# DefaultRui/VLN-VER

Measured on AMD Instinct MI355X. Metric: viewpoints/sec (multi-view->voxel fwd+bwd), vocc.py config, higher is better.
Workload: dtype bf16

## Files before the change

### vln-ver_amd/csrc/ver_wgrad.hip

```cpp
#include <cstdlib>
#include "ver_common.h"

namespace {
typedef __bf16 bf16x8 __attribute__((ext_vector_type(8)));
typedef float f32x16 __attribute__((ext_vector_type(16)));
typedef short s16x4 __attribute__((ext_vector_type(4)));
typedef short s16x8 __attribute__((ext_vector_type(8)));
typedef __attribute__((address_space(3))) s16x4 lds_s16x4;
typedef __attribute__((address_space(3))) void lds_void;

constexpr int kTile = 256;
constexpr int kSlabRows = 16;
constexpr int kSlabBytes = 2 * kSlabRows * kTile * 2;
constexpr int kRing = 8;
constexpr int kLdsBytes = kRing * kSlabBytes;

typedef int i32x2 __attribute__((ext_vector_type(2)));
typedef int i32x4 __attribute__((ext_vector_type(4)));

template <int OFF>
__device__ __forceinline__ i32x2 tr_read(int addr) {
    i32x2 v;
    asm volatile("ds_read_b64_tr_b16 %0, %1 offset:%2" : "=v"(v) : "v"(addr), "n"(OFF) : "memory");
    return v;
}
__device__ __forceinline__ bf16x8 frag(i32x2 lo, i32x2 hi) {
    return __builtin_bit_cast(bf16x8, (i32x4)__builtin_shufflevector(lo, hi, 0, 1, 2, 3));
}

struct WgradArgs {
    const __bf16* A;
    const __bf16* G;
    float* ws;
    long lda, ldg, M, Mc;
    int S, Ka, N, tiles_n, T;
    void* out;
    long ldo;
    int out_bf16;
    const __bf16* lattice;
    long lattice_bytes;
    const __bf16* cst;
    long cst_bytes;
    int B, H, W, C, P, CW, ncst, nseg;
    int seg_start[65];
    signed char kind[64], dz[64], dy[64], dx[64];
};

constexpr int kOutsideW = (int)0x80000000;
template <int L>
__device__ __forceinline__ int wcell_off(const WgradArgs& t, int b, int zl, int y, int x, int dz) {
    if ((unsigned)y >= (unsigned)t.H || (unsigned)x >= (unsigned)t.W) return kOutsideW;
    const int j = dz >> 1;
    int v;
    if (L == 0)
        v = ((b * 4 + zl + dz) * t.H + y) * t.W + x;
    else if (L == 2)
        v = ((((b * 2 + zl) * t.H + y) * t.W + x) << 1) + j;
    else
        v = (((((((y & 1) << 1 | (x & 1)) * t.B + b) * 2 + zl) * (t.H >> 1) + (y >> 1)) * (t.W >> 1) + (x >> 1)) << 1) + j;
    return v * t.C * 2;
}

struct WTapLane {
    int taddr;
    int boff;
    int bstep;
    int pend;
    int tend;
    int rows_left;
    int vo;
};

template <int L>
__device__ __forceinline__ int wtap_table_entry(const WgradArgs& t, int seg, int pos) {
    if (seg < 0) return kOutsideW;
    if (t.kind[seg]) return (pos * t.ncst + t.dz[seg]) * t.CW * 2;
    const int hw = t.H * t.W;
    const int zl = pos / hw, rem = pos - zl * hw;
    const int y = rem / t.W, x = rem - y * t.W;
    return wcell_off<L>(t, 0, zl, y + t.dy[seg], x + t.dx[seg], t.dz[seg]);
}

__device__ __forceinline__ int lds_read_b32(int addr) {
    int v;
    asm volatile("ds_read_b32 %0, %1" : "=v"(v) : "v"(addr) : "memory");
    return v;
}

__device__ __forceinline__ void wtap_step(const WgradArgs& t, WTapLane& tl, int tfetched) {
    tl.boff += tl.pend;
    tl.rows_left -= kSlabRows;
    tl.vo = tl.rows_left > 0 ? (int)((unsigned)tfetched + (unsigned)tl.boff) : kOutsideW;
    tl.taddr += 4 * kSlabRows;
    tl.pend = 0;
    if (tl.taddr >= tl.tend) tl.taddr -= 4 * t.P, tl.pend = tl.bstep;
}

struct WgradLane {
    int offA0, offA1, offB0, offB1;
    int voA, voG;
    int stepA, stepG;
    int dmaoff;
};

template <int SLOT>
__device__ __forceinline__ void read_slab(const WgradLane& c, i32x2 (&al)[4], i32x2 (&ah)[4], i32x2 (&bl)[2], i32x2 (&bh)[2]) {
    constexpr int SB = (SLOT & 3) * kSlabBytes;
    constexpr int UP = SLOT >= 4 ? 65536 : 0;
    const int a0 = c.offA0 + UP, a1 = c.offA1 + UP, b0 = c.offB0 + UP, b1 = c.offB1 + UP;
    al[0] = tr_read<SB>(a0);
    ah[0] = tr_read<SB + 512>(a0);
    bl[0] = tr_read<SB>(b0);
    bh[0] = tr_read<SB + 512>(b0);
    al[1] = tr_read<SB>(a1);
    ah[1] = tr_read<SB + 512>(a1);
    bl[1] = tr_read<SB>(b1);
    bh[1] = tr_read<SB + 512>(b1);
    al[2] = tr_read<SB + 1024>(a0);
    ah[2] = tr_read<SB + 1536>(a0);
    al[3] = tr_read<SB + 1024>(a1);
    ah[3] = tr_read<SB + 1536>(a1);
}

template <int PS, int KP, int PF, int IMPL>
__device__ __forceinline__ void phase(char* lds, f32x16 (&acc)[4][2], const WgradLane& c, __amdgpu_buffer_rsrc_t ra,
                                      __amdgpu_buffer_rsrc_t rg, unsigned& soA, unsigned& soG, const WgradArgs& t, WTapLane& tl) {
    i32x2 al[KP][4], ah[KP][4], bl[KP][2], bh[KP][2];
    int tnext = 0;
    read_slab<PS * KP>(c, al[0], ah[0], bl[0], bh[0]);
    if constexpr (KP == 2) read_slab<PS * KP + 1>(c, al[KP - 1], ah[KP - 1], bl[KP - 1], bh[KP - 1]);
#pragma unroll
    for (int u = 0; u < KP; ++u) {
        const int ds = (PS * KP + u + PF) % kRing;
        if constexpr (IMPL < 0) {
            __builtin_amdgcn_raw_ptr_buffer_load_lds(ra, (lds_void*)(lds + ds * kSlabBytes + c.dmaoff), 16, c.voA, (int)soA, 0, 0);
        } else {
            static_assert(IMPL < 0 || KP == 1, "implicit A: one slab per phase");
            __builtin_amdgcn_raw_ptr_buffer_load_lds(ra, (lds_void*)(lds + ds * kSlabBytes + c.dmaoff), 16, tl.vo, 0, 0, 0);
            tnext = lds_read_b32(tl.taddr);
        }
        __builtin_amdgcn_raw_ptr_buffer_load_lds(rg, (lds_void*)(lds + ds * kSlabBytes + kSlabBytes / 2 + c.dmaoff), 16, c.voG, (int)soG, 0, 0);
        soA += (unsigned)c.stepA;
        soG += (unsigned)c.stepG;
    }
    asm volatile("s_waitcnt vmcnt(%0)" ::"n"(2 * (PF - KP)) : "memory");
    __builtin_amdgcn_s_barrier();
    asm volatile("s_waitcnt lgkmcnt(0)"
                 : "+v"(al[0][0]), "+v"(ah[0][0]), "+v"(al[0][1]), "+v"(ah[0][1]), "+v"(al[0][2]), "+v"(ah[0][2]), "+v"(al[0][3]),
                   "+v"(ah[0][3]), "+v"(bl[0][0]), "+v"(bh[0][0]), "+v"(bl[0][1]), "+v"(bh[0][1]), "+v"(tnext)
                 :
                 : "memory");

    if constexpr (KP == 2)
        asm volatile(""
                     : "+v"(al[KP - 1][0]), "+v"(ah[KP - 1][0]), "+v"(al[KP - 1][1]), "+v"(ah[KP - 1][1]), "+v"(al[KP - 1][2]),
                       "+v"(ah[KP - 1][2]), "+v"(al[KP - 1][3]), "+v"(ah[KP - 1][3]), "+v"(bl[KP - 1][0]), "+v"(bh[KP - 1][0]),
                       "+v"(bl[KP - 1][1]), "+v"(bh[KP - 1][1])
                     :
                     : "memory");
    bf16x8 a[KP][4], b[KP][2];
#pragma unroll
    for (int u = 0; u < KP; ++u) {
#pragma unroll
        for (int i = 0; i < 4; ++i) a[u][i] = frag(al[u][i], ah[u][i]);
        b[u][0] = frag(bl[u][0], bh[u][0]);
        b[u][1] = frag(bl[u][1], bh[u][1]);
    }
    __builtin_amdgcn_sched_barrier(0);
    __builtin_amdgcn_s_setprio(1);
#pragma unroll
    for (int u = 0; u < KP; ++u)
#pragma unroll
        for (int it = 0; it < 4; ++it)
#pragma unroll
            for (int jt = 0; jt < 2; ++jt)
                acc[it][jt] = __builtin_amdgcn_mfma_f32_32x32x16_bf16(a[u][it], b[u][jt], acc[it][jt], 0, 0, 0);
    __builtin_amdgcn_s_setprio(0);
    __builtin_amdgcn_sched_barrier(0);
    if constexpr (IMPL >= 0) {
        wtap_step(t, tl, tnext);
        __builtin_amdgcn_sched_barrier(0);
    }
    __builtin_amdgcn_s_barrier();
}

template <int PS, int KP, int PF, int IMPL>
__device__ __forceinline__ void phases_from(int left, char* lds, f32x16 (&acc)[4][2], const WgradLane& c,
                                            __amdgpu_buffer_rsrc_t ra, __amdgpu_buffer_rsrc_t rg, unsigned& soA, unsigned& soG,
                                            const WgradArgs& t, WTapLane& tl) {
    if constexpr (PS < kRing / KP) {
        if (left > PS * KP) {
            phase<PS, KP, PF, IMPL>(lds, acc, c, ra, rg, soA, soG, t, tl);
            phases_from<PS + 1, KP, PF, IMPL>(left, lds, acc, c, ra, rg, soA, soG, t, tl);
        }
    }
}

template <int KP, int PF, int IMPL>
__device__ __forceinline__ void wgrad_body(const WgradArgs& p) {
    static_assert(PF >= KP && PF + (KP == 1 ? 2 : 4) <= kRing, "prefetch distance against the ring (WAR on the slot)");
    extern __shared__ __attribute__((aligned(1024))) char lds[];
    const int tid = threadIdx.x, lane = tid & 63;
    const int wave = __builtin_amdgcn_readfirstlane(tid >> 6);
    const int wr = wave >> 2, wc = wave & 3;
    int chunk, tile;
    {
        const int b = blockIdx.x;
        if ((p.S & 7) == 0) {
            const int xcd = b & 7, idx = b >> 3;
            chunk = xcd + 8 * (idx / p.T);
            tile = idx % p.T;
        } else {
            chunk = b / p.T;
            tile = b % p.T;
        }
    }
    const int mt = tile / p.tiles_n, nt = tile - mt * p.tiles_n;
    const long row0 = (long)chunk * p.Mc;
    const long rows = max(0L, min(p.Mc, p.M - row0));
    const int nslab = (int)((rows + kSlabRows * KP - 1) / (kSlabRows * KP)) * KP;

    const __bf16* ab = IMPL < 0 ? p.A + row0 * p.lda + (long)mt * kTile : nullptr;
    const __bf16* gb = p.G + row0 * p.ldg + (long)nt * kTile;
    const long abytes = ((p.M - row0 - 1) * p.lda + p.Ka - (long)mt * kTile) * 2;
    const long gbytes = ((p.M - row0 - 1) * p.ldg + p.N - (long)nt * kTile) * 2;
    const __amdgpu_buffer_rsrc_t rg = __builtin_amdgcn_make_buffer_rsrc((void*)gb, 0, (int)max(0L, min(gbytes, 0xFFFFFFFFL)), 0x00020000);
    WgradLane c;
    const int prow = lane >> 3, pch = (lane & 7) ^ (((prow >> 1) & 1) << 2);
    WTapLane tl = {};
    bool a_cst = false;
    if constexpr (IMPL >= 0) {
        int* tables = reinterpret_cast<int*>(lds + kLdsBytes);
        auto seg_of = [&](int col0) {
            int seg = -1;
            for (int i = 0; i < p.nseg; ++i)
                if (col0 >= p.seg_start[i] && col0 < p.seg_start[i + 1]) seg = i;
            return seg;
        };
        for (int q = 0; q < 4; ++q) {
            const int seg = seg_of(mt * kTile + 64 * q);
            for (int i = tid; i < p.P; i += 512) tables[q * p.P + i] = wtap_table_entry<IMPL>(p, seg, i);
        }
        __syncthreads();
        const int col0 = mt * kTile + 64 * (wave & 3);
        const int seg = seg_of(col0);
        a_cst = seg >= 0 && p.kind[seg];
        const long r = row0 + 8 * (wave >> 2) + prow;
        const int b0 = (int)(r / p.P), pos0 = (int)(r - (long)b0 * p.P);
        tl.bstep = a_cst ? 0 : (IMPL == 3 ? p.H * p.W : 4 * p.H * p.W) * p.C * 2;
        tl.boff = b0 * tl.bstep + (seg < 0 ? 0 : (col0 - p.seg_start[seg]) * 2) + pch * 16;
        const int lbase = (int)(uintptr_t)(__attribute__((address_space(3))) char*)(lds + kLdsBytes) + (wave & 3) * p.P * 4;
        tl.tend = lbase + 4 * p.P;
        tl.taddr = lbase + 4 * pos0;
        tl.pend = 0;
        tl.rows_left = (int)min(min(p.M, row0 + p.Mc) - r, 0x7FFFFFF0L) + kSlabRows;
        int t0 = lds_read_b32(tl.taddr);
        asm volatile("s_waitcnt lgkmcnt(0)" : "+v"(t0)::"memory");
        wtap_step(p, tl, t0);
    }
    const __amdgpu_buffer_rsrc_t ra =
        IMPL < 0 ? __builtin_amdgcn_make_buffer_rsrc((void*)ab, 0, (int)max(0L, min(abytes, 0xFFFFFFFFL)), 0x00020000)
                 : __builtin_amdgcn_make_buffer_rsrc((void*)(a_cst ? p.cst : p.lattice), 0,
                                                     (int)max(0L, min(a_cst ? p.cst_bytes : p.lattice_bytes, 0x7FFFFFFFL)), 0x00020000);
    c.voA = (int)(((8 * (wave >> 2) + prow) * p.lda + 64 * (wave & 3)) * 2) + pch * 16;
    c.voG = (int)(((8 * (wave >> 2) + prow) * p.ldg + 64 * (wave & 3)) * 2) + pch * 16;
    c.stepA = (int)(kSlabRows * p.lda * 2);
    c.stepG = (int)(kSlabRows * p.ldg * 2);
    c.dmaoff = wave * 1024;
    unsigned soA = 0, soG = 0;

    {
        const int q = lane >> 4, cl = lane & 15;
        const int lowch = (2 * (q & 1) + ((cl & 3) >> 1)) ^ (((cl >> 3) & 1) << 2);
        const int lbase = (int)(uintptr_t)(__attribute__((address_space(3))) char*)lds;
        const int rowoff = lbase + ((q >> 1) * 32 + (cl >> 2)) * 128 + lowch * 16 + (cl & 1) * 8;
        c.offA0 = rowoff + 2 * wr * 1024;
        c.offA1 = c.offA0 ^ 64;
        c.offB0 = rowoff + wc * 1024 + kSlabBytes / 2;
        c.offB1 = c.offB0 ^ 64;
    }

    f32x16 acc[4][2];
#pragma unroll
    for (int it = 0; it < 4; ++it)
#pragma unroll
        for (int jt = 0; jt < 2; ++jt)
#pragma unroll
            for (int r = 0; r < 16; ++r) acc[it][jt][r] = 0.0f;

#pragma unroll
    for (int s = 0; s < PF; ++s) {
        if constexpr (IMPL < 0) {
            __builtin_amdgcn_raw_ptr_buffer_load_lds(ra, (lds_void*)(lds + s * kSlabBytes + c.dmaoff), 16, c.voA, (int)soA, 0, 0);
        } else {
            __builtin_amdgcn_raw_ptr_buffer_load_lds(ra, (lds_void*)(lds + s * kSlabBytes + c.dmaoff), 16, tl.vo, 0, 0, 0);
            int tn = lds_read_b32(tl.taddr);
            asm volatile("s_waitcnt lgkmcnt(0)" : "+v"(tn)::"memory");
            wtap_step(p, tl, tn);
        }
        __builtin_amdgcn_raw_ptr_buffer_load_lds(rg, (lds_void*)(lds + s * kSlabBytes + kSlabBytes / 2 + c.dmaoff), 16, c.voG, (int)soG, 0, 0);
        soA += (unsigned)c.stepA;
        soG += (unsigned)c.stepG;
    }
    asm volatile("s_waitcnt vmcnt(%0)" ::"n"(2 * (PF - KP)) : "memory");
    __builtin_amdgcn_s_barrier();
    if (wr == 1) __builtin_amdgcn_s_barrier();

    int s = 0;
    for (; s + kRing <= nslab; s += kRing) phases_from<0, KP, PF, IMPL>(kRing, lds, acc, c, ra, rg, soA, soG, p, tl);
    phases_from<0, KP, PF, IMPL>(nslab - s, lds, acc, c, ra, rg, soA, soG, p, tl);
    if (wr == 0) __builtin_amdgcn_s_barrier();
    asm volatile("s_waitcnt vmcnt(0)" ::: "memory");

    const int i0 = mt * kTile + 128 * wr + 4 * (lane >> 5), j0 = nt * kTile + 64 * wc + (lane & 31);
    if (p.S == 1 && p.out) {
#pragma unroll
        for (int it = 0; it < 4; ++it)
#pragma unroll
            for (int jt = 0; jt < 2; ++jt) {
                const int j = j0 + 32 * jt;
#pragma unroll
                for (int r = 0; r < 16; ++r) {
                    const int i = i0 + 32 * it + (r & 3) + 8 * (r >> 2);
                    if (i < p.Ka && j < p.N) {
                        if (p.out_bf16)
                            reinterpret_cast<__bf16*>(p.out)[(long)i * p.ldo + j] = (__bf16)acc[it][jt][r];
                        else
                            reinterpret_cast<float*>(p.out)[(long)i * p.ldo + j] = acc[it][jt][r];
                    }
                }
            }
        return;
    }
    float* out = p.ws + (long)chunk * p.Ka * p.N;
#pragma unroll
    for (int it = 0; it < 4; ++it)
#pragma unroll
        for (int jt = 0; jt < 2; ++jt) {
            const int j = j0 + 32 * jt;
#pragma unroll
            for (int r = 0; r < 16; ++r) {
                const int i = i0 + 32 * it + (r & 3) + 8 * (r >> 2);
                if (i < p.Ka && j < p.N) out[(long)i * p.N + j] = acc[it][jt][r];
            }
        }
}

template <int KP, int PF>
__global__ __launch_bounds__(512) void k_wgrad_tn(WgradArgs p) {
    wgrad_body<KP, PF, -1>(p);
}

template <int L, int PF>
__global__ __launch_bounds__(512) void k_wgrad_tn_seg(WgradArgs p) {
    wgrad_body<1, PF, L>(p);
}

template <typename OT>
__global__ __launch_bounds__(256) void k_wgrad_reduce(const float* __restrict__ ws, OT* __restrict__ out, long ldo, int S,
                                                      int Ka, int N) {
    const long n4 = (long)Ka * N / 4;
    const long stride = (long)Ka * N;
    for (long e = blockIdx.x * 256L + threadIdx.x; e < n4; e += (long)gridDim.x * 256) {
        float4 acc = *reinterpret_cast<const float4*>(ws + 4 * e);
        for (int s = 1; s < S; ++s) {
            const float4 v = *reinterpret_cast<const float4*>(ws + s * stride + 4 * e);
            acc.x += v.x;
            acc.y += v.y;
            acc.z += v.z;
            acc.w += v.w;
        }
        const long i = (4 * e) / N, j = (4 * e) - i * N;
        OT* o = out + i * ldo + j;
        if constexpr (sizeof(OT) == 4) {
            *reinterpret_cast<float4*>(o) = acc;
        } else {
            typedef __bf16 bf16x4 __attribute__((ext_vector_type(4)));
            bf16x4 v;
            v.x = (__bf16)acc.x;
            v.y = (__bf16)acc.y;
            v.z = (__bf16)acc.z;
            v.w = (__bf16)acc.w;
            *reinterpret_cast<bf16x4*>(o) = v;
        }
    }
}

long max_chunk_rows(long ld) {
    if (ld <= 0) return 45000;
    const long rows = (0xFFFFFFFFL / (ld * 2)) - 16 * kRing - 2 * kSlabRows - 1;
    return rows < 45000 ? (rows > 2 * kSlabRows ? rows : 2 * kSlabRows) : 45000;
}

int pick_splits(long M, int Ka, int N, long ld = 0) {
    const long cap = max_chunk_rows(ld);
    const long tiles = (long)((Ka + kTile - 1) / kTile) * ((N + kTile - 1) / kTile);
    static const int cand[] = {1, 2, 3, 4, 6, 8, 12, 16, 24, 32, 48, 64};
    int best = 0;
    double best_us = 0.0;
    for (int s : cand) {
        if ((M + s - 1) / s > cap) continue;
        if (s > 1 && M / s < 256) break;
        if (M > 32768 && s % 8) continue;
        const long rounds = (tiles * s + 255) / 256;
        const double slabs = (double)((M + s - 1) / s + 15) / 16.0;
        double us = (double)rounds * (slabs * 0.37 + 8.0) + (s == 1 ? 0.25 : (double)s) * (double)Ka * (double)N * 8.0 / 3.0e6;
        if (s % 8 == 0) us *= 0.97;
        if (!best || us < best_us) {
            best = s;
            best_us = us;
        }
    }
    if (!best) {
        best = 64;
        while (best < 65536 && (M + best - 1) / best > cap) best *= 2;
    }
    return best;
}

template <int KP, int PF>
void launch_tn(const WgradArgs& p, int blocks, hipStream_t st, hipError_t& e) {
    auto kern = k_wgrad_tn<KP, PF>;
    e = hipFuncSetAttribute((const void*)kern, hipFuncAttributeMaxDynamicSharedMemorySize, kLdsBytes);
    if (e == hipSuccess) hipLaunchKernelGGL(kern, dim3((unsigned)blocks), dim3(512), kLdsBytes, st, p);
}
template <int L, int PF>
void launch_tn_segments_pf(const WgradArgs& p, int blocks, hipStream_t st, hipError_t& e) {
    const int ldsb = kLdsBytes + 4 * p.P * 4;
    e = hipFuncSetAttribute((const void*)k_wgrad_tn_seg<L, PF>, hipFuncAttributeMaxDynamicSharedMemorySize, ldsb);
    if (e == hipSuccess) hipLaunchKernelGGL((k_wgrad_tn_seg<L, PF>), dim3((unsigned)blocks), dim3(512), ldsb, st, p);
}

template <int L>
void launch_tn_segments(const WgradArgs& p, int blocks, hipStream_t st, hipError_t& e) {
    static const int pf = [] {
        const char* v = getenv("VER_WGRAD_SEG_PF");
        return v ? atoi(v) : 3;
    }();
    if (pf == 4) launch_tn_segments_pf<L, 4>(p, blocks, st, e);
    else if (pf == 5) launch_tn_segments_pf<L, 5>(p, blocks, st, e);
    else if (pf == 6) launch_tn_segments_pf<L, 6>(p, blocks, st, e);
    else launch_tn_segments_pf<L, 3>(p, blocks, st, e);
}
}

extern "C" int ver_wgrad_tn_splits(long M, int Ka, int N) {
    if (M <= 0 || Ka <= 0 || N <= 0) return 1;
    return pick_splits(M, Ka, N);
}

extern "C" int ver_wgrad_tn_splits_ld(long M, int Ka, int N, long ld) {
    if (M <= 0 || Ka <= 0 || N <= 0) return 1;
    return pick_splits(M, Ka, N, ld);
}

extern "C" long ver_wgrad_tn_workspace(long M, int Ka, int N, int splits) {
    if (Ka <= 0 || N <= 0) return 0;
    if (splits <= 0) splits = ver_wgrad_tn_splits(M, Ka, N);
    return (long)splits * Ka * N * (long)sizeof(float);
}

extern "C" int ver_wgrad_tn(const void* a, long lda, const void* g, long ldg, long M, int Ka, int N, void* out, long ldo,
                            int out_dtype, int splits, int flags, void* workspace, long workspace_bytes, void* stream) {
    hipStream_t st = (hipStream_t)stream;
    VER_REQUIRE(M >= 0 && Ka > 0 && N > 0, VER_EINVAL, "ver_wgrad_tn: bad sizes M=%ld Ka=%d N=%d", M, Ka, N);
    VER_REQUIRE(out && workspace && ((a && g) || M == 0), VER_EINVAL, "ver_wgrad_tn: null pointer argument");
    VER_REQUIRE(out_dtype == VER_F32 || out_dtype == VER_BF16, VER_EINVAL, "ver_wgrad_tn: out_dtype %d", out_dtype);
    VER_REQUIRE(lda >= Ka && ldg >= N && ldo >= N, VER_EINVAL, "ver_wgrad_tn: row pitch smaller than the row");
    VER_REQUIRE(lda % 8 == 0 && ldg % 8 == 0 && ((uintptr_t)a & 15) == 0 && ((uintptr_t)g & 15) == 0, VER_EUNSUPPORTED,
                "ver_wgrad_tn: operands must be 16-byte aligned with row pitches that are multiples of 8 elements");
    VER_REQUIRE(N % 4 == 0 && ldo % 4 == 0 && ((uintptr_t)out & 15) == 0, VER_EUNSUPPORTED,
                "ver_wgrad_tn: N and the output pitch must be multiples of 4");
    const int S = splits > 0 ? splits : pick_splits(M, Ka, N, lda > ldg ? lda : ldg);
    VER_REQUIRE(S <= 65536, VER_EINVAL, "ver_wgrad_tn: %d row chunks", S);
    const long Mc = ((M + S - 1) / S + 2 * kSlabRows - 1) / (2 * kSlabRows) * (2 * kSlabRows);
    VER_REQUIRE((Mc + 16 * kRing) * (lda > ldg ? lda : ldg) * 2 < 0xFFFFFFFFL, VER_EUNSUPPORTED,
                "ver_wgrad_tn: a row chunk exceeds the 4-GiB range of a buffer offset (more splits)");
    VER_REQUIRE(workspace_bytes >= (long)S * Ka * N * (long)sizeof(float), VER_EINVAL, "ver_wgrad_tn: workspace of %ld bytes, %ld needed",
                workspace_bytes, (long)S * Ka * N * (long)sizeof(float));
    WgradArgs p = {};
    p.A = (const __bf16*)a;
    p.G = (const __bf16*)g;
    p.ws = (float*)workspace;
    p.lda = lda;
    p.ldg = ldg;
    p.M = M;
    p.Mc = Mc;
    p.S = S;
    p.Ka = Ka;
    p.N = N;
    p.tiles_n = (N + kTile - 1) / kTile;
    p.T = ((Ka + kTile - 1) / kTile) * p.tiles_n;
    const bool direct = S == 1 && M > 0;
    p.out = direct ? out : nullptr;
    p.ldo = ldo;
    p.out_bf16 = out_dtype == VER_BF16;
    hipError_t e = hipSuccess;
    if (M > 0) {
        switch (flags & 15) {
            case 4: launch_tn<1, 4>(p, p.T * S, st, e); break;
            case 5: launch_tn<1, 5>(p, p.T * S, st, e); break;
            case 6: launch_tn<1, 6>(p, p.T * S, st, e); break;
            case 8 + 2: launch_tn<2, 2>(p, p.T * S, st, e); break;
            case 8 + 4: launch_tn<2, 4>(p, p.T * S, st, e); break;
            default: launch_tn<1, 3>(p, p.T * S, st, e); break;
        }
        if (e != hipSuccess) return ver_fail(VER_ELAUNCH, "ver_wgrad_tn: LDS attribute: %s", hipGetErrorString(e));
    } else if (int zrc = ver_zero_async(workspace, (size_t)S * Ka * N * sizeof(float), st)) {
        return zrc;
    }
    if (direct) return ver_check_launch("ver_wgrad_tn");
    const long n4 = (long)Ka * N / 4;
    long grid = (n4 + 255) / 256;
    if (grid > 8192) grid = 8192;
    if (out_dtype == VER_F32)
        hipLaunchKernelGGL(k_wgrad_reduce<float>, dim3((unsigned)grid), dim3(256), 0, st, (const float*)workspace, (float*)out, ldo, S, Ka, N);
    else
        hipLaunchKernelGGL(k_wgrad_reduce<__bf16>, dim3((unsigned)grid), dim3(256), 0, st, (const float*)workspace, (__bf16*)out, ldo, S, Ka, N);
    return ver_check_launch("ver_wgrad_tn");
}

extern "C" int ver_wgrad_tn_segments(const void* lattice, int layout, int B, int H, int W, int C, const int* taps, int nseg,
                                     const void* cst, int ncst, int cw, const void* g, long ldg, int N, void* out, long ldo,
                                     int out_dtype, int splits, void* workspace, long workspace_bytes, void* stream) {
    hipStream_t st = (hipStream_t)stream;
    VER_REQUIRE(B >= 0 && H > 0 && W > 0 && C > 0 && N > 0 && nseg > 0, VER_EINVAL, "ver_wgrad_tn_segments: bad sizes");
    VER_REQUIRE(layout == 0 || layout == 2 || layout == 3, VER_EINVAL, "ver_wgrad_tn_segments: layout %d (0 plain, 2 z-split, 3 planar z-split)", layout);
    VER_REQUIRE(layout != 3 || (H % 2 == 0 && W % 2 == 0), VER_EINVAL, "ver_wgrad_tn_segments: planar needs even H, W");
    VER_REQUIRE(out && workspace && ((lattice && g && taps) || B == 0), VER_EINVAL, "ver_wgrad_tn_segments: null pointer argument");
    VER_REQUIRE(out_dtype == VER_F32 || out_dtype == VER_BF16, VER_EINVAL, "ver_wgrad_tn_segments: out_dtype %d", out_dtype);
    VER_REQUIRE(nseg <= 64, VER_EUNSUPPORTED, "ver_wgrad_tn_segments: %d segments (at most 64)", nseg);
    VER_REQUIRE(C % 64 == 0 && (cst == nullptr || (ncst > 0 && ncst <= 64 && cw > 0 && cw % 64 == 0 && ((uintptr_t)cst & 15) == 0)),
                VER_EUNSUPPORTED, "ver_wgrad_tn_segments: segment widths (C = %d, pattern blocks of %d) must be multiples of 64", C, cw);
    const long M = (long)B * 2 * H * W, lbytes = (long)B * 4 * H * W * C * 2;
    const int P = 2 * H * W;
    VER_REQUIRE(P >= kSlabRows && P <= 2048 && lbytes < 0x7FFFFFFFL, VER_EUNSUPPORTED,
                "ver_wgrad_tn_segments: %d rows per viewpoint / a source lattice of %ld bytes (16 <= rows <= 2048: four offset tables "
                "next to the 128-KB ring in LDS; below 2 GiB)", P, lbytes);
    VER_REQUIRE(ldg >= N && ldo >= N && ldg % 8 == 0 && ((uintptr_t)g & 15) == 0 && ((uintptr_t)lattice & 15) == 0, VER_EUNSUPPORTED,
                "ver_wgrad_tn_segments: g must be 16-byte aligned with a row pitch that is a multiple of 8 elements");
    VER_REQUIRE(N % 4 == 0 && ldo % 4 == 0 && ((uintptr_t)out & 15) == 0, VER_EUNSUPPORTED,
                "ver_wgrad_tn_segments: N and the output pitch must be multiples of 4");
    WgradArgs p = {};
    long Ka = 0;
    for (int i = 0; i < nseg; ++i) {
        const int dz = taps[3 * i], dy = taps[3 * i + 1], dx = taps[3 * i + 2];
        p.seg_start[i] = (int)Ka;
        if (dz < 0) {
            VER_REQUIRE(cst && -1 - dz < ncst, VER_EINVAL, "ver_wgrad_tn_segments: segment %d names pattern block %d of %d", i, -1 - dz, cst ? ncst : 0);
            p.kind[i] = 1, p.dz[i] = (signed char)(-1 - dz);
            Ka += cw;
        } else {
            VER_REQUIRE((dz == 0 || dz == 2) && dy >= -64 && dy <= 64 && dx >= -64 && dx <= 64, VER_EINVAL,
                        "ver_wgrad_tn_segments: tap %d = (%d, %d, %d): dz must be 0 or 2", i, dz, dy, dx);
            p.kind[i] = 0, p.dz[i] = (signed char)dz, p.dy[i] = (signed char)dy, p.dx[i] = (signed char)dx;
            Ka += C;
        }
    }
    p.seg_start[nseg] = (int)Ka;
    VER_REQUIRE(Ka < 0x7FFFFFFFL, VER_EUNSUPPORTED, "ver_wgrad_tn_segments: %ld columns", Ka);
    const int S = splits > 0 ? splits : pick_splits(M, (int)Ka, N, ldg);
    VER_REQUIRE(S <= 65536, VER_EINVAL, "ver_wgrad_tn_segments: %d row chunks", S);
    const long Mc = ((M + S - 1) / S + 2 * kSlabRows - 1) / (2 * kSlabRows) * (2 * kSlabRows);
    VER_REQUIRE((Mc + 16 * kRing) * ldg * 2 < 0xFFFFFFFFL, VER_EUNSUPPORTED,
                "ver_wgrad_tn_segments: a row chunk exceeds the 4-GiB range of a buffer offset (more splits)");
    VER_REQUIRE(workspace_bytes >= (long)S * Ka * N * (long)sizeof(float), VER_EINVAL, "ver_wgrad_tn_segments: workspace of %ld bytes, %ld needed",
                workspace_bytes, (long)S * Ka * N * (long)sizeof(float));
    p.A = nullptr;
    p.G = (const __bf16*)g;
    p.ws = (float*)workspace;
    p.lda = 0;
    p.ldg = ldg;
    p.M = M;
    p.Mc = Mc;
    p.S = S;
    p.Ka = (int)Ka;
    p.N = N;
    p.tiles_n = (N + kTile - 1) / kTile;
    p.T = (int)((Ka + kTile - 1) / kTile) * p.tiles_n;
    const bool direct = S == 1 && M > 0;
    p.out = direct ? out : nullptr;
    p.ldo = ldo;
    p.out_bf16 = out_dtype == VER_BF16;
    p.lattice = (const __bf16*)lattice;
    p.lattice_bytes = lbytes;
    p.cst = (const __bf16*)cst;
    p.cst_bytes = cst ? (long)P * ncst * cw * 2 : 0;
    p.B = B, p.H = H, p.W = W, p.C = C, p.P = P, p.CW = cw, p.ncst = ncst, p.nseg = nseg;
    hipError_t e = hipSuccess;
    if (M > 0) {
        if (layout == 0) launch_tn_segments<0>(p, p.T * S, st, e);
        else if (layout == 2) launch_tn_segments<2>(p, p.T * S, st, e);
        else launch_tn_segments<3>(p, p.T * S, st, e);
        if (e != hipSuccess) return ver_fail(VER_ELAUNCH, "ver_wgrad_tn_segments: LDS attribute: %s", hipGetErrorString(e));
    } else if (int zrc = ver_zero_async(workspace, (size_t)S * Ka * N * sizeof(float), st)) {
        return zrc;
    }
    if (direct) return ver_check_launch("ver_wgrad_tn_segments");
    const long n4 = Ka * N / 4;
    long grid = (n4 + 255) / 256;
    if (grid > 8192) grid = 8192;
    if (out_dtype == VER_F32)
        hipLaunchKernelGGL(k_wgrad_reduce<float>, dim3((unsigned)grid), dim3(256), 0, st, (const float*)workspace, (float*)out, ldo, S, (int)Ka, N);
    else
        hipLaunchKernelGGL(k_wgrad_reduce<__bf16>, dim3((unsigned)grid), dim3(256), 0, st, (const float*)workspace, (__bf16*)out, ldo, S, (int)Ka, N);
    return ver_check_launch("ver_wgrad_tn_segments");
}

extern "C" int ver_wgrad_tn_segments_splits(int B, int H, int W, long Ka, int N, long ldg) {
    const long M = (long)B * 2 * H * W;
    if (M <= 0 || Ka <= 0 || N <= 0) return 1;
    return pick_splits(M, (int)Ka, N, ldg);
}
```

Before: 715.7.

## Fuse split-K reduction into wgrad kernel via per-tile atomic tickets

Replaces the separate split-K reduce launch with an in-kernel last-block reduction. Each block writes its partial tile to the workspace, takes a ticket on a per-tile counter, and the block that arrives last sums all S partials and writes the final output, then resets the counter. This removes one kernel launch and lets the reduction overlap with the tail of the GEMM. In exchange it adds fence and atomic overhead, serialises the reduce work onto one block per tile, and uses a host-side ticket pool that is allocated lazily.

After: 697.6. 2.5% lower.

```diff
diff --git a/vln-ver_amd/csrc/ver_wgrad.hip b/vln-ver_amd/csrc/ver_wgrad.hip
--- a/vln-ver_amd/csrc/ver_wgrad.hip
+++ b/vln-ver_amd/csrc/ver_wgrad.hip
@@ -1,4 +1,5 @@
 #include <cstdlib>
+#include <mutex>
 #include "ver_common.h"
 
 namespace {
@@ -37,6 +38,7 @@
     void* out;
     long ldo;
     int out_bf16;
+    unsigned* tickets;
     const __bf16* lattice;
     long lattice_bytes;
     const __bf16* cst;
@@ -192,6 +194,74 @@
         if (left > PS * KP) {
             phase<PS, KP, PF, IMPL>(lds, acc, c, ra, rg, soA, soG, t, tl);
             phases_from<PS + 1, KP, PF, IMPL>(left, lds, acc, c, ra, rg, soA, soG, t, tl);
+        }
+    }
+}
+
+__device__ __forceinline__ float4 add4(float4 a, float4 b) { return make_float4(a.x + b.x, a.y + b.y, a.z + b.z, a.w + b.w); }
+
+__device__ __forceinline__ void reduce_tile(const WgradArgs& p, char* lds, int tile, int mt, int nt) {
+    const int tid = threadIdx.x;
+    int* last = reinterpret_cast<int*>(lds);
+    asm volatile("s_waitcnt vmcnt(0)" ::: "memory");
+    __syncthreads();
+    if (tid == 0) {
+        __builtin_amdgcn_fence(__ATOMIC_RELEASE, "agent");
+        asm volatile("s_waitcnt vmcnt(0)" ::: "memory");
+        const unsigned ticket = __hip_atomic_fetch_add(p.tickets + tile, 1u, __ATOMIC_RELAXED, __HIP_MEMORY_SCOPE_AGENT);
+        const bool mine = ticket == (unsigned)(p.S - 1);
+        if (mine) {
+            __builtin_amdgcn_fence(__ATOMIC_ACQUIRE, "agent");
+            asm volatile("s_waitcnt vmcnt(0)" ::: "memory");
+            __hip_atomic_store(p.tickets + tile, 0u, __ATOMIC_RELAXED, __HIP_MEMORY_SCOPE_AGENT);
+        }
+        *last = mine;
+    }
+    __syncthreads();
+    if (!*last) return;
+
+    const int rows = min(kTile, p.Ka - mt * kTile), cols4 = min(kTile, p.N - nt * kTile) >> 2;
+    const long stride = (long)p.Ka * p.N;
+    const int c4 = tid & 63;
+    if (c4 >= cols4) return;
+    const float* src = p.ws + (long)mt * kTile * p.N + nt * kTile + 4 * c4;
+    for (int r = tid >> 6; r < rows; r += 16) {
+        const bool two = r + 8 < rows;
+        const float* s0 = src + (long)r * p.N;
+        const float* s1 = two ? s0 + 8L * p.N : s0;
+        float4 a0 = *reinterpret_cast<const float4*>(s0), a1 = *reinterpret_cast<const float4*>(s1);
+        int s = 1;
+        for (; s + 4 <= p.S; s += 4) {
+            float4 v0[4], v1[4];
+#pragma unroll
+            for (int u = 0; u < 4; ++u) {
+                v0[u] = *reinterpret_cast<const float4*>(s0 + (s + u) * stride);
+                v1[u] = *reinterpret_cast<const float4*>(s1 + (s + u) * stride);
+            }
+#pragma unroll
+            for (int u = 0; u < 4; ++u) a0 = add4(a0, v0[u]), a1 = add4(a1, v1[u]);
+        }
+        for (; s < p.S; ++s) {
+            a0 = add4(a0, *reinterpret_cast<const float4*>(s0 + s * stride));
+            a1 = add4(a1, *reinterpret_cast<const float4*>(s1 + s * stride));
+        }
+        const long o0 = (long)(mt * kTile + r) * p.ldo + nt * kTile + 4 * c4;
+#pragma unroll
+        for (int h = 0; h < 2; ++h) {
+            if (h && !two) break;
+            const float4 a = h ? a1 : a0;
+            const long o = o0 + h * 8L * p.ldo;
+            if (p.out_bf16) {
+                typedef __bf16 bf16x4 __attribute__((ext_vector_type(4)));
+                bf16x4 v;
+                v.x = (__bf16)a.x;
+                v.y = (__bf16)a.y;
+                v.z = (__bf16)a.z;
+                v.w = (__bf16)a.w;
+                *reinterpret_cast<bf16x4*>(reinterpret_cast<__bf16*>(p.out) + o) = v;
+            } else {
+                *reinterpret_cast<float4*>(reinterpret_cast<float*>(p.out) + o) = a;
+            }
         }
     }
 }
@@ -344,6 +414,7 @@
                 if (i < p.Ka && j < p.N) out[(long)i * p.N + j] = acc[it][jt][r];
             }
         }
+    if (p.tickets) reduce_tile(p, lds, tile, mt, nt);
 }
 
 template <int KP, int PF>
@@ -441,6 +512,60 @@
     else if (pf == 5) launch_tn_segments_pf<L, 5>(p, blocks, st, e);
     else if (pf == 6) launch_tn_segments_pf<L, 6>(p, blocks, st, e);
     else launch_tn_segments_pf<L, 3>(p, blocks, st, e);
+}
+constexpr int kTicketRing = 1 << 16;
+constexpr int kMaxDevices = 64;
+
+unsigned* take_tickets(int T, hipStream_t st) {
+    struct Pool {
+        unsigned* base = nullptr;
+        int cursor = 0;
+        bool failed = false;
+    };
+    static std::mutex mu;
+    static Pool pools[kMaxDevices];
+    int dev = -1;
+    if (T > kTicketRing || hipGetDevice(&dev) != hipSuccess || dev < 0 || dev >= kMaxDevices) return nullptr;
+    std::lock_guard<std::mutex> lock(mu);
+    Pool& pool = pools[dev];
+    if (!pool.base) {
+        hipStreamCaptureStatus cap = hipStreamCaptureStatusNone;
+        if (pool.failed || hipStreamIsCapturing(st, &cap) != hipSuccess || cap != hipStreamCaptureStatusNone) return nullptr;
+        void* mem = nullptr;
+        if (hipMalloc(&mem, kTicketRing * sizeof(unsigned)) != hipSuccess) {
+            (void)hipGetLastError();
+            pool.failed = true;
+            return nullptr;
+        }
+        if (ver_zero_async(mem, kTicketRing * sizeof(unsigned), st) != 0 || hipStreamSynchronize(st) != hipSuccess) {
+            (void)hipGetLastError();
+            (void)hipFree(mem);
+            pool.failed = true;
+            return nullptr;
+        }
+        pool.base = (unsigned*)mem;
+    }
+    if (pool.cursor + T > kTicketRing) pool.cursor = 0;
+    unsigned* t = pool.base + pool.cursor;
+    pool.cursor += T;
+    return t;
+}
+
+void set_result_path(WgradArgs& p, void* out, hipStream_t st) {
+    p.tickets = p.S > 1 && p.M > 0 ? take_tickets(p.T, st) : nullptr;
+    p.out = (p.S == 1 && p.M > 0) || p.tickets ? out : nullptr;
+}
+
+int finish_product(const WgradArgs& p, void* out, int out_dtype, hipStream_t st, const char* what) {
+    if (p.out) return ver_check_launch(what);
+    const long n4 = (long)p.Ka * p.N / 4;
+    long grid = (n4 + 255) / 256;
+    if (grid > 8192) grid = 8192;
+    if (out_dtype == VER_F32)
+        hipLaunchKernelGGL(k_wgrad_reduce<float>, dim3((unsigned)grid), dim3(256), 0, st, (const float*)p.ws, (float*)out, p.ldo, p.S, p.Ka, p.N);
+    else
+        hipLaunchKernelGGL(k_wgrad_reduce<__bf16>, dim3((unsigned)grid), dim3(256), 0, st, (const float*)p.ws, (__bf16*)out, p.ldo, p.S, p.Ka, p.N);
+    return ver_check_launch(what);
 }
 }
 
@@ -491,10 +616,9 @@
     p.N = N;
     p.tiles_n = (N + kTile - 1) / kTile;
     p.T = ((Ka + kTile - 1) / kTile) * p.tiles_n;
-    const bool direct = S == 1 && M > 0;
-    p.out = direct ? out : nullptr;
     p.ldo = ldo;
     p.out_bf16 = out_dtype == VER_BF16;
+    set_result_path(p, out, st);
     hipError_t e = hipSuccess;
     if (M > 0) {
         switch (flags & 15) {
@@ -509,15 +633,7 @@
     } else if (int zrc = ver_zero_async(workspace, (size_t)S * Ka * N * sizeof(float), st)) {
         return zrc;
     }
-    if (direct) return ver_check_launch("ver_wgrad_tn");
-    const long n4 = (long)Ka * N / 4;
-    long grid = (n4 + 255) / 256;
-    if (grid > 8192) grid = 8192;
-    if (out_dtype == VER_F32)
-        hipLaunchKernelGGL(k_wgrad_reduce<float>, dim3((unsigned)grid), dim3(256), 0, st, (const float*)workspace, (float*)out, ldo, S, Ka, N);
-    else
-        hipLaunchKernelGGL(k_wgrad_reduce<__bf16>, dim3((unsigned)grid), dim3(256), 0, st, (const float*)workspace, (__bf16*)out, ldo, S, Ka, N);
-    return ver_check_launch("ver_wgrad_tn");
+    return finish_product(p, out, out_dtype, st, "ver_wgrad_tn");
 }
 
 extern "C" int ver_wgrad_tn_segments(const void* lattice, int layout, int B, int H, int W, int C, const int* taps, int nseg,
@@ -578,10 +694,9 @@
     p.N = N;
     p.tiles_n = (N + kTile - 1) / kTile;
     p.T = (int)((Ka + kTile - 1) / kTile) * p.tiles_n;
-    const bool direct = S == 1 && M > 0;
-    p.out = direct ? out : nullptr;
     p.ldo = ldo;
     p.out_bf16 = out_dtype == VER_BF16;
+    set_result_path(p, out, st);
     p.lattice = (const __bf16*)lattice;
     p.lattice_bytes = lbytes;
     p.cst = (const __bf16*)cst;
@@ -596,15 +711,7 @@
     } else if (int zrc = ver_zero_async(workspace, (size_t)S * Ka * N * sizeof(float), st)) {
         return zrc;
     }
-    if (direct) return ver_check_launch("ver_wgrad_tn_segments");
-    const long n4 = Ka * N / 4;
-    long grid = (n4 + 255) / 256;
-    if (grid > 8192) grid = 8192;
-    if (out_dtype == VER_F32)
-        hipLaunchKernelGGL(k_wgrad_reduce<float>, dim3((unsigned)grid), dim3(256), 0, st, (const float*)workspace, (float*)out, ldo, S, (int)Ka, N);
-    else
-        hipLaunchKernelGGL(k_wgrad_reduce<__bf16>, dim3((unsigned)grid), dim3(256), 0, st, (const float*)workspace, (__bf16*)out, ldo, S, (int)Ka, N);
-    return ver_check_launch("ver_wgrad_tn_segments");
+    return finish_product(p, out, out_dtype, st, "ver_wgrad_tn_segments");
 }
 
 extern "C" int ver_wgrad_tn_segments_splits(int B, int H, int W, long Ka, int N, long ldg) {
```
